# Bazs/structure_from_motion

Hardware: NVIDIA B200
Metric: hyp x point evals/sec (fp64) (higher is better)
Workload: dtype f64

## Files before the change

include/sfm_b200.h:

```cpp
#ifndef SFM_B200_H
#define SFM_B200_H

#include <stdint.h>

#ifdef __cplusplus
extern "C" {
#endif

typedef struct sfm_ctx sfm_ctx;

enum sfm_status {
    SFM_OK = 0,
    SFM_ERR_ARG = -1,
    SFM_ERR_CUDA = -2,
    SFM_ERR_STATE = -3,
    SFM_ERR_NO_DEVICE = -4
};

enum sfm_aggregation { SFM_AGG_SUM = 0, SFM_AGG_SQUARE = 1, SFM_AGG_MEAN = 2, SFM_AGG_RMS = 3 };
enum sfm_selection { SFM_SELECT_MIN_ERROR = 0, SFM_SELECT_MAX_INLIERS = 1, SFM_SELECT_MSAC = 2 };
enum sfm_score_variant { SFM_SCORE_SCREEN = 0, SFM_SCORE_FULL = 1, SFM_SCORE_SCREEN32 = 2, SFM_SCORE_AUTO = 3 };

int sfm_version(void);
const char *sfm_last_error(void);
int sfm_device_count(void);
int sfm_create(int device, sfm_ctx **out);
int sfm_destroy(sfm_ctx *ctx);
int sfm_set_stream(sfm_ctx *ctx, void *cuda_stream);
int sfm_use_default_stream(sfm_ctx *ctx);
int sfm_synchronize(sfm_ctx *ctx);
int sfm_set_score_variant(sfm_ctx *ctx, int variant, int hyps_per_thread, int group);
int sfm_host_alloc(uint64_t bytes, void **out);
int sfm_host_free(void *p);

int sfm_mt_shuffle_table(uint32_t *state625, int64_t n, int64_t h, int32_t *table, int64_t perm_at,
                         int32_t *perm_out);
// ... 22 lines not shown

typedef struct sfm_best {
    double err;
    int64_t index;
    int32_t count_extra;
    int32_t reserved;
    int64_t num_invalid;
    int64_t first_invalid;
    double E[9];
    int32_t sample[8];
} sfm_best;
int sfm_get_best(sfm_ctx *ctx, sfm_best *out);
int sfm_set_winner(sfm_ctx *ctx, int64_t local_index, const double *E);
int sfm_near_ties(sfm_ctx *ctx, double rel_tol, int64_t cap, int64_t *idx_out, int64_t *count);
int sfm_get_rescored(sfm_ctx *ctx, int64_t *count);
int sfm_inlier_mask(sfm_ctx *ctx, double threshold, uint8_t *mask, double *sed);

int sfm_ransac_essential(sfm_ctx *ctx, double threshold, double min_extra, int aggregation,
                         int selection, sfm_best *best, uint8_t *mask, double *sed);

int sfm_fit_homography(sfm_ctx *ctx, double *H_out, uint8_t *valid_out);
int sfm_ransac_homography(sfm_ctx *ctx, double threshold, double min_extra, int aggregation, int selection,
                          sfm_best *best, uint8_t *mask, double *err, int32_t *count_extra_h, double *err_h);
int sfm_homography_mask(sfm_ctx *ctx, const double *H, double threshold, uint8_t *mask, double *err);

typedef struct sfm_poses {
    double R[4][9];
    double t[4][3];
    double sv[3];
    int64_t counts[4];
// ... 107 lines not shown
```

structure_from_motion_b200/_native.py:

```python
from __future__ import annotations

import ctypes as C
import os
import threading

import numpy as np

_HERE = os.path.dirname(os.path.abspath(__file__))
LIB_PATH = os.environ.get("SFM_B200_LIB") or os.path.join(_HERE, "libsfm_b200.so")

AGG = {"sum": 0, "square": 1, "mean": 2, "rms": 3}
SELECT = {"min_error": 0, "max_inliers": 1, "msac": 2}
VARIANT = {"screen": 0, "full": 1, "screen32": 2, "auto": 3}


class NativeUnavailableError(RuntimeError):
    """libsfm_b200.so is missing / not loadable, or there is no B200 to run it on."""


class NativeError(RuntimeError):
    """A C-ABI call returned a non-zero status."""


class Best(C.Structure):
    _fields_ = [("err", C.c_double), ("index", C.c_int64), ("count_extra", C.c_int32),
                ("reserved", C.c_int32), ("num_invalid", C.c_int64), ("first_invalid", C.c_int64),
                ("E", C.c_double * 9), ("sample", C.c_int32 * 8)]

# ... 34 lines not shown
    "sfm_set_table": (C.c_int, [_P, _P, C.c_int64]),
    "sfm_sample_device": (C.c_int, [_P, C.c_uint64, C.c_uint64, C.c_int64, C.c_int64]),
    "sfm_get_table": (C.c_int, [_P, _P, C.c_int64, C.c_int64]),
    "sfm_upload_pairs": (C.c_int, [_P, _P, _P, _P, _P, C.c_int64, C.c_int64, _P]),
    "sfm_upload_pairs_async": (C.c_int, [_P, _P, _P, _P, _P, C.c_int64, C.c_int64, _P]),
    "sfm_upload_pairs_d": (C.c_int, [_P, _P, _P, _P, _P, C.c_int64, C.c_int64, _P]),
    "sfm_get_normalised": (C.c_int, [_P, _P, C.c_int64]),
    "sfm_fit": (C.c_int, [_P, _P, _P, _P]),
    "sfm_set_models": (C.c_int, [_P, _P, _P, C.c_int64]),
    "sfm_get_models": (C.c_int, [_P, C.c_int64, C.c_int64, _P, _P]),
    "sfm_score": (C.c_int, [_P, C.c_double, C.c_double, C.c_int, C.c_int, C.c_int, C.c_int64, _P, _P, _P, _P]),
    "sfm_get_best": (C.c_int, [_P, C.POINTER(Best)]),
    "sfm_set_winner": (C.c_int, [_P, C.c_int64, _P]),
    "sfm_near_ties": (C.c_int, [_P, C.c_double, C.c_int64, _P, C.POINTER(C.c_int64)]),
    "sfm_get_rescored": (C.c_int, [_P, C.POINTER(C.c_int64)]),
    "sfm_inlier_mask": (C.c_int, [_P, C.c_double, _P, _P]),
    "sfm_ransac_essential": (C.c_int, [_P, C.c_double, C.c_double, C.c_int, C.c_int, C.POINTER(Best), _P, _P]),
    "sfm_fit_homography": (C.c_int, [_P, _P, _P]),
    "sfm_ransac_homography": (C.c_int, [_P, C.c_double, C.c_double, C.c_int, C.c_int, C.POINTER(Best), _P, _P, _P, _P]),
    "sfm_homography_mask": (C.c_int, [_P, _P, C.c_double, _P, _P]),
    "sfm_decompose_essential": (C.c_int, [_P, _P, C.POINTER(Poses)]),
    "sfm_recover_pose": (C.c_int, [_P, _P, _P, _P, _P, _P, C.c_int64, C.c_int64, C.c_double, C.POINTER(Poses), _P]),
    "sfm_recover_pose_pixels": (C.c_int, [_P, _P, _P, _P, _P, _P, _P, C.c_int64, C.c_int64, C.c_double,
                                          C.POINTER(Poses), _P]),
    "sfm_triangulate": (C.c_int, [_P, _P, _P, _P, _P, _P, _P, C.c_int64, C.c_int64, _P]),
    "sfm_pose_and_triangulate": (C.c_int, [_P, C.c_double, C.c_double, C.POINTER(Poses), C.c_int64,
                                           C.POINTER(C.c_int64), _P, _P, _P]),
    "sfm_two_view": (C.c_int, [_P, C.c_double, C.c_double, C.c_int, C.c_int, C.c_double, C.POINTER(Best), C.POINTER(Poses),
                               C.c_int64, C.POINTER(C.c_int64), _P, _P, _P, _P, _P]),
    "sfm_two_view_async": (C.c_int, [_P, C.c_double, C.c_double, C.c_int, C.c_int, C.c_double, _P, _P]),
# ... 229 lines not shown
    def set_winner(self, local_index, E=None):
        Ea = None if E is None else _f64(E).reshape(9)
        self._ck(self.lib.sfm_set_winner(self.h, int(local_index), _ptr(Ea)), "sfm_set_winner")

    def near_ties(self, rel_tol=1e-12, cap=64):
        idx = np.empty(cap, dtype=np.int64)
        n = C.c_int64(0)
        self._ck(self.lib.sfm_near_ties(self.h, float(rel_tol), int(cap), _ptr(idx), C.byref(n)), "sfm_near_ties")
        return np.sort(idx[:min(int(n.value), cap)]), int(n.value)

    def rescored(self) -> int:
        n = C.c_int64(0)
        self._ck(self.lib.sfm_get_rescored(self.h, C.byref(n)), "sfm_get_rescored")
        return int(n.value)

    def inlier_mask(self, threshold, want_sed=True):
        mask = np.empty(self.n, dtype=np.uint8)
        sed = np.empty(self.n, dtype=np.float64) if want_sed else None
        self._ck(self.lib.sfm_inlier_mask(self.h, float(threshold), _ptr(mask), _ptr(sed)), "sfm_inlier_mask")
        return mask.astype(bool), sed

    def ransac_essential(self, threshold, min_extra=0.0, aggregation="rms", selection="min_error",
                         want_mask=True, want_sed=True, mask_out=None, sed_out=None):
        b = Best()
        mask = mask_out if mask_out is not None else (np.empty(self.n, dtype=np.uint8) if want_mask else None)
        sed = sed_out if sed_out is not None else (np.empty(self.n, dtype=np.float64) if want_sed else None)
        self._ck(self.lib.sfm_ransac_essential(self.h, float(threshold), float(min_extra), AGG[aggregation],
                                               SELECT[selection], C.byref(b), _ptr(mask), _ptr(sed)),
                 "sfm_ransac_essential")
        return b, mask, sed
# ... 447 lines not shown
```

structure_from_motion_b200/csrc/sfm_api.cu:

```cuda
#include "../../include/sfm_b200.h"

#include <dlfcn.h>

#include <cmath>
#include <cstdarg>
#include <cstdio>
#include <cstdlib>
#include <cstring>
#include <string>
#include <vector>

#include "sfm_device.cuh"
#include "sfm_fit.cuh"
#include "sfm_linalg.cuh"
#include "sfm_score.cuh"
#include "sfm_homography.cuh"
#include "sfm_pose.cuh"
#include "sfm_tail.cuh"
#include "sfm_misc.cuh"
#include "sfm_match.cuh"
#include "sfm_harris.cuh"
#include "sfm_select.cuh"

using namespace sfm;

static_assert(sizeof(Corr) == 32, "Corr must be 32 bytes");
static_assert(sizeof(PoseSet) == sizeof(sfm_poses), "PoseSet/sfm_poses layout mismatch");
static_assert(sizeof(SelectRecord) == SFM_RECORD_BYTES, "SelectRecord / SFM_RECORD_BYTES mismatch");
static_assert(sizeof(ModelScores) == sizeof(sfm_model_scores), "ModelScores / sfm_model_scores layout mismatch");

// ... 54 lines not shown
enum { T_UPLOAD = 0, T_SAMPLE, T_FIT, T_SCORE, T_SELECT, T_MASK, T_POSE, T_TRI, T_COUNT };

}

struct sfm_ctx {
    int device = 0;
    int sm_count = 148;
    cudaStream_t own_stream = nullptr, stream = nullptr;
    Buf raw, pts, offsets, Ks, table, E, valid, eig;
    Buf acc, count_extra, S1, S2, err, blocks, best, invalid, winnerE, spts, bounds, fitflag, record, merged, rows, blockinv;
    Buf m_img, m_feat, m_W, m_ss, m_ok, m_S, m_out;
    Buf h_img, h_gx, h_gy, h_corner, h_alive, h_key, h_idx, h_small, h_xy;
    Buf mask, sed, poses, pass, X, idx, scan, tmp, tailstate, num, winrec, bout;
    Buf planes, hK;
    Buf selstate, selpp;
    long long n = 0, h = 0, npairs = 1;
    long long first_len = 0;
    long long raw_stride = 1;
    bool batched = false, has_pts = false, has_table = false, has_models = false, has_score = false;
    bool models_h = false;
    int hscore_occ = 0;
    bool table_pending = false;
    unsigned long long smp_seed = 0, smp_stream = 0;
    long long smp_offset = 0;
    bool acc_clean = false;
    size_t acc_planes_for = 0;
    double Kstage[9] = {0};
    double hstage[18] = {0};
    double sstage[27] = {0};
    const void* occ_fn[4] = {nullptr, nullptr, nullptr, nullptr};
// ... 157 lines not shown
        c->ev_used[i] = false;
    }
    CU(cudaFuncSetAttribute(k_fit, cudaFuncAttributeMaxDynamicSharedMemorySize,
                            (int)(kFitThreads * kFitSmemDoubles * sizeof(double))));
    *out = c;
    return 0;
}

int sfm_destroy(sfm_ctx* c) {
    if (!c) return 0;
    cudaSetDevice(c->device);
    cudaStreamSynchronize(c->stream);
    Buf* bufs[] = {&c->raw, &c->pts, &c->offsets, &c->Ks, &c->table, &c->E, &c->valid, &c->eig, &c->acc,
                   &c->count_extra, &c->S1, &c->S2, &c->err, &c->blocks, &c->best,
                   &c->invalid, &c->winnerE, &c->record, &c->merged, &c->rows, &c->blockinv, &c->mask, &c->sed, &c->poses, &c->pass, &c->X, &c->idx,
                   &c->planes, &c->hK, &c->selstate, &c->selpp,
                   &c->scan, &c->tmp, &c->gathered, &c->tailstate, &c->num, &c->winrec, &c->bout, &c->spts, &c->bounds, &c->fitflag,
                   &c->m_img, &c->m_feat, &c->m_W, &c->m_ss, &c->m_ok, &c->m_S, &c->m_out,
                   &c->h_img, &c->h_gx, &c->h_gy, &c->h_corner, &c->h_alive, &c->h_key, &c->h_idx, &c->h_small, &c->h_xy};
    for (Buf* b : bufs) b->release();
    for (int i = 0; i < T_COUNT; ++i) {
        cudaEventDestroy(c->ev0[i]);
        cudaEventDestroy(c->ev1[i]);
    }
    sfm_nccl_destroy(c);
    if (c->hpin) cudaFreeHost(c->hpin);
    cudaStreamDestroy(c->own_stream);
    delete c;
    return 0;
}

// ... 5 lines not shown

int sfm_use_default_stream(sfm_ctx* c) {
    if (int r = use(c)) return r;
    c->stream = cudaStreamLegacy;
    return 0;
}

int sfm_synchronize(sfm_ctx* c) {
    if (int r = use(c)) return r;
    CU(cudaStreamSynchronize(c->stream));
    return 0;
}

int sfm_set_score_variant(sfm_ctx* c, int variant, int hpt, int group) {
    if (!c) return fail(SFM_ERR_ARG, "null context");
    if (variant != SFM_SCORE_SCREEN && variant != SFM_SCORE_FULL && variant != SFM_SCORE_SCREEN32 && variant != SFM_SCORE_AUTO)
        return fail(SFM_ERR_ARG, "bad variant %d", variant);
    int nh = hpt ? hpt : c->hpt, ng = group ? group : c->group;
    if (!hpt && (variant == SFM_SCORE_SCREEN32) != (c->variant == SFM_SCORE_SCREEN32)) {
        nh = variant == SFM_SCORE_SCREEN32 ? 4 : 2;
        ng = variant == SFM_SCORE_SCREEN32 ? 8 : 16;
    }
    if (!score_kernel(variant == SFM_SCORE_AUTO ? SFM_SCORE_SCREEN : variant, nh, ng) ||
        (variant == SFM_SCORE_AUTO && !score_kernel(SFM_SCORE_FULL, nh, ng)))
        return fail(SFM_ERR_ARG, "unsupported combination: hyps_per_thread %d, group %d", nh, ng);
    c->variant = variant;
    c->hpt = nh;
    c->group = ng;
    return 0;
}

int sfm_host_alloc(uint64_t bytes, void** out) {
    if (!out) return fail(SFM_ERR_ARG, "out is null");
    CU(cudaMallocHost(out, bytes ? bytes : 1));
    return 0;
}
int sfm_host_free(void* p) {
    if (p) CU(cudaFreeHost(p));
// ... 53 lines not shown

int sfm_get_table(sfm_ctx* c, int32_t* table, int64_t first, int64_t h) {
    if (int r = use(c)) return r;
    if (!c->has_table || first < 0 || h < 0 || first + h > c->h * c->npairs)
        return fail(SFM_ERR_STATE, "no table rows [%lld, %lld)", (long long)first, (long long)(first + h));
    if (int r = ensure_table(c)) return r;
    CU(cudaMemcpyAsync(table, c->table.as<int32_t>() + 8 * first, (size_t)h * 32, cudaMemcpyDeviceToHost, c->stream));
    CU(cudaStreamSynchronize(c->stream));
    return 0;
}

static int normalise_from(sfm_ctx* c, const double* xa, const double* ya, const double* xb, const double* yb,
                          int64_t stride, int64_t n, int64_t max_len) {
    if (int r = c->pts.reserve((size_t)n * sizeof(Corr))) return r;
    if (int r = c->bounds.reserve(16)) return r;
    CU(cudaMemsetAsync(c->bounds.p, 0, 16, c->stream));
    dim3 grid((unsigned)((max_len + 255) / 256), (unsigned)c->npairs);
    k_normalise<<<grid, 256, 0, c->stream>>>(xa, ya, xb, yb, stride, n,
                                             c->batched ? c->offsets.as<long long>() : nullptr,
                                             c->Ks.as<double>(), c->pts.as<Corr>(), c->bounds.as<unsigned long long>());
    return check_launch(c, "k_normalise");
}

static int stage_coords(sfm_ctx* c, double* d, const double* xa, const double* ya, const double* xb, const double* yb,
                        int64_t stride, int64_t n, const double* s[4]) {
    if (stride == 1) {
        const double* src[4] = {xa, ya, xb, yb};
        for (int k = 0; k < 4; ++k)
            CU(cudaMemcpyAsync(d + (size_t)k * n, src[k], (size_t)n * sizeof(double), cudaMemcpyHostToDevice, c->stream));
        s[0] = d; s[1] = d + n; s[2] = d + 2 * n; s[3] = d + 3 * n;
    } else if (stride == 2 && ya == xa + 1 && yb == xb + 1) {
        CU(cudaMemcpyAsync(d, xa, (size_t)n * 2 * sizeof(double), cudaMemcpyHostToDevice, c->stream));
        CU(cudaMemcpyAsync(d + 2 * n, xb, (size_t)n * 2 * sizeof(double), cudaMemcpyHostToDevice, c->stream));
        s[0] = d; s[1] = d + 1; s[2] = d + 2 * n; s[3] = d + 2 * n + 1;
    } else {
        return fail(SFM_ERR_ARG, "unsupported layout: stride must be 1 (four arrays) or 2 (two interleaved [n][2] arrays)");
// ... 31 lines not shown
        const double* src[4] = {xa, ya, xb, yb};
        for (int k = 0; k < 4; ++k) {
            CU(cudaMemcpy2DAsync(d + (size_t)k * n, sizeof(double), src[k], (size_t)stride * sizeof(double),
                                 sizeof(double), (size_t)n, cudaMemcpyDeviceToDevice, c->stream));
            s[k] = d + (size_t)k * n;
        }
        c->raw_stride = stride = 1;
    } else if (int r = stage_raw(c, xa, ya, xb, yb, stride, n, s)) {
        return r;
    }
    if (int r = c->Ks.reserve(9 * sizeof(double))) return r;
    memcpy(c->Khost, K, sizeof c->Khost);
    CU(cudaMemcpyAsync(c->Ks.p, c->Khost, 9 * sizeof(double), cudaMemcpyHostToDevice, c->stream));
    c->n = n;
    if (int r = normalise_from(c, s[0], s[1], s[2], s[3], stride, n, n)) return r;
    c->toc(T_UPLOAD);
    if (sync) CU(cudaStreamSynchronize(c->stream));
    c->has_pts = true;
    c->has_table = c->has_models = c->has_score = false;
    c->table_pending = false;
    c->winner_set = false;
    return 0;
}

int sfm_upload_pairs(sfm_ctx* c, const double* xa, const double* ya, const double* xb, const double* yb,
                     int64_t stride, int64_t n, const double* K) {
    return upload_pairs_impl(c, xa, ya, xb, yb, stride, n, K, false, true);
}

int sfm_upload_pairs_async(sfm_ctx* c, const double* xa, const double* ya, const double* xb, const double* yb,
// ... 199 lines not shown
        if (int r = ensure_table(c)) return r;
    if (agg < 0 || agg > 3) return fail(SFM_ERR_ARG, "bad aggregation %d", agg);
    if (mode < 0 || mode > 2) return fail(SFM_ERR_ARG, "bad selection %d", mode);
    const bool skip_k2 = !(thr >= 0.0) || thr > 1e100;
    const int force_rescore = (thr > 1e100) ? 1 : 0;
    const long long h = c->h, P = c->npairs;
    const int hpt = (c->variant == SFM_SCORE_SCREEN32 && thr > 1e6) ? 2 : c->hpt;
    const int G = (c->variant == SFM_SCORE_SCREEN32 && thr > 1e6) ? 16 : c->group;
    const long long hblocks = (h + 32ll * hpt - 1) / (32ll * hpt);
    const size_t H = (size_t)h * P;
    if (int r = reserve_selection(c, h, P)) return r;
    int e2 = 0;
    if (thr > 0.0 && !skip_k2) (void)frexp(thr, &e2);
    if (e2 < -400) e2 = -400;
    const bool autov = c->variant == SFM_SCORE_AUTO;
    int variant = autov ? SFM_SCORE_SCREEN : c->variant;
    if (variant == SFM_SCORE_SCREEN32 && thr > 1e6) variant = SFM_SCORE_SCREEN;
    const bool f32 = variant == SFM_SCORE_SCREEN32;
    const bool screen = variant != SFM_SCORE_FULL;
    double thr_pre = f32 ? thr * kThr32Factor : (screen ? thr * (1.0 + 1e-9) : thr * (1.0 + 1e-9) + 1e-22);
    if (f32 && thr_pre < 1e-24) thr_pre = 1e-24;
    if (screen && thr_pre < 1e-280) thr_pre = 1e-280;
    const double s_scale = sqrt(thr_pre);
    const double scale1 = ldexp(1.0, 63 - e2), scale2 = ldexp(1.0, 63 - 2 * e2);
    unsigned long long* acc_dev = nullptr;
    {
        const void* fn = score_kernel(variant, hpt, G);
        if (!fn) return fail(SFM_ERR_ARG, "unsupported scoring configuration (variant %d, hpt %d, group %d)", variant, hpt, G);
        const size_t smem_one = (size_t)kScoreWarps * score_warp_smem(hpt, false);
        const size_t smem_two = (size_t)kScoreWarps * score_warp_smem(hpt, true);
        const size_t smem_both = smem_one > smem_two ? smem_one : smem_two;
// ... 15 lines not shown
        if (int r = occupancy(fn, smem, &occ)) return r;
#ifndef SFM_AUTO_SINGLE
#define SFM_AUTO_SINGLE 1
#endif
        const void* fn_auto = nullptr;
        if (autov && SFM_AUTO_SINGLE) {
            if (hpt == 2 && G == 16) fn_auto = reinterpret_cast<const void*>(&k_score_auto<2, 16>);
            if (hpt == 4 && G == 8) fn_auto = reinterpret_cast<const void*>(&k_score_auto<4, 8>);
        }
        if (fn_auto)
            if (int r = occupancy(fn_auto, smem_both, &occ)) return r;
        const void* fn_full = (autov && !fn_auto) ? score_kernel(SFM_SCORE_FULL, hpt, G) : nullptr;
        int occ_full = 0;
        if (fn_full)
            if (int r = occupancy(fn_full, smem_two, &occ_full)) return r;
        const long long grid_blocks = (long long)c->sm_count * occ;
        constexpr int items_per_warp = 32;
        const ItemSplit sp = split_items(grid_blocks * kScoreWarps * items_per_warp, hblocks * P, max_len, kTile);
        const long long chunk = sp.chunk, nsplit = sp.nsplit;
        const long long total_items = hblocks * nsplit * P;
        if (int r = c->acc.reserve(H * kAccWords * 8 + acc_tail_bytes(P))) return r;
        const long long npts = c->n;
        if (f32) { if (int r = c->spts.reserve((size_t)npts * sizeof(Corr32))) return r; }
        else if (screen) { if (int r = c->spts.reserve((size_t)npts * sizeof(Corr))) return r; }
        ScoreArgs a;
        a.pts = c->pts.as<Corr>();
        a.spts = screen ? c->spts.p : c->pts.p;
        a.bounds = c->bounds.as<double>();
        a.s = s_scale;
        a.kappa_coef = kKappaCoef * (1.0 + thr);
// ... 6 lines not shown
        a.thr = thr;
        a.thr_pre = thr_pre;
        a.scale1 = scale1;
        a.scale2 = scale2;
        a.sums = sums;
        a.chunk = chunk;
        a.hblocks = (int)hblocks;
        a.nsplit = (int)nsplit;
        a.total_items = total_items;
        a.htotal = (long long)H;
        a.acc = c->acc.as<unsigned long long>();
        a.work_counter = reinterpret_cast<unsigned*>(a.acc + H * kAccWords);
        char* tailp = reinterpret_cast<char*>(a.acc + H * kAccWords);
        a.mode_flag = autov ? reinterpret_cast<const int*>(tailp + 32) : nullptr;
        acc_dev = a.acc;
        c->tic(T_SCORE);
        if (int r = clear_acc(c, H, P)) return r;
        if (f32 && !skip_k2) {
            k_screen_pts32<<<(unsigned)((npts + 255) / 256), 256, 0, c->stream>>>(c->pts.as<Corr>(), npts, 1.0 / s_scale,
                                                                                  reinterpret_cast<Corr32*>(c->spts.p));
            if (int r = check_launch(c, "k_screen_pts32")) return r;
        }
        else if (screen && !skip_k2) {
            PilotArgs pa;
            pa.E = c->E.as<double>();
            pa.h = h;
            pa.plen = c->batched ? c->first_len : c->n;
            pa.thr_pre = thr_pre;
            pa.counters = reinterpret_cast<unsigned*>(tailp + 16);
            pa.mode_flag = autov ? reinterpret_cast<int*>(tailp + 32) : nullptr;
            CU(chain_launch(c, k_screen_pts64, dim3((unsigned)((npts + 255) / 256)), dim3(256), 0, c->pts.as<Corr>(), npts,
                            1.0 / s_scale, reinterpret_cast<Corr*>(c->spts.p), pa));
            if (int r = check_launch(c, "k_screen_pts64")) return r;
        }
        const long long want_blocks = (total_items + kScoreWarps - 1) / kScoreWarps;
        const long long launch_blocks = grid_blocks < want_blocks ? grid_blocks : want_blocks;
        void* kargs[] = {(void*)&a};
        if (!skip_k2 && fn_auto) {
            ScoreArgs a2 = a;
            a2.thr_pre = thr * (1.0 + 1e-9) + 1e-22;
            a2.spts = c->pts.p;
            void* kargs2[] = {(void*)&a, (void*)&a2};
            CU(chain_launch_ptr(c, fn_auto, dim3((unsigned)launch_blocks), dim3(kScoreThreads), smem_both, kargs2));
            if (int r = check_launch(c, "k_score_auto")) return r;
        } else if (!skip_k2) {
            CU(chain_launch_ptr(c, fn, dim3((unsigned)launch_blocks), dim3(kScoreThreads), smem, kargs));
            if (int r = check_launch(c, "k_score")) return r;
            if (fn_full) {
                ScoreArgs a2 = a;
                a2.thr_pre = thr * (1.0 + 1e-9) + 1e-22;
                a2.spts = c->pts.p;
                const long long gb2 = (long long)c->sm_count * occ_full;
                const long long lb2 = gb2 < want_blocks ? gb2 : want_blocks;
                void* kargs2[] = {(void*)&a2};
                CU(chain_launch_ptr(c, fn_full, dim3((unsigned)lb2), dim3(kScoreThreads), smem_two, kargs2));
                if (int r = check_launch(c, "k_score")) return r;
            }
        }
        c->toc(T_SCORE);
    }

    return finalise_launch(c, MODEL_E, thr, min_extra, agg, mode, use_table, idx_offset, sums, e2, force_rescore, acc_dev);
}

int sfm_score(sfm_ctx* c, double thr, double min_extra, int agg, int mode, int use_table, int64_t idx_offset,
              int32_t* count_extra, double* S1, double* S2, double* err) {
    if (int r = use(c)) return r;
    if (c->batched) return fail(SFM_ERR_STATE, "sfm_score is a single-pair call; use sfm_batch_ransac");
    if (int r = score_launch(c, thr, min_extra, agg, mode, use_table != 0, idx_offset, c->n, S1 || S2)) return r;
    const size_t H = (size_t)c->h;
    if (count_extra) CU(cudaMemcpyAsync(count_extra, c->count_extra.p, H * 4, cudaMemcpyDeviceToHost, c->stream));
    if (S1) CU(cudaMemcpyAsync(S1, c->S1.p, H * 8, cudaMemcpyDeviceToHost, c->stream));
    if (S2) CU(cudaMemcpyAsync(S2, c->S2.p, H * 8, cudaMemcpyDeviceToHost, c->stream));
    if (err) CU(cudaMemcpyAsync(err, c->err.p, H * 8, cudaMemcpyDeviceToHost, c->stream));
    CU(cudaStreamSynchronize(c->stream));
    return 0;
// ... 38 lines not shown
    if (int r = c->tmp.reserve((size_t)cap * 8 + 16)) return r;
    unsigned* cnt = c->tmp.as<unsigned>();
    long long* out = reinterpret_cast<long long*>(c->tmp.as<char>() + 16);
    CU(cudaMemsetAsync(cnt, 0, 16, c->stream));
    const int blocks = (int)((c->h + 255) / 256 < 4 * c->sm_count ? (c->h + 255) / 256 : 4 * c->sm_count);
    k_near_ties<<<blocks, 256, 0, c->stream>>>(c->err.as<double>(), c->h, c->record.as<SelectRecord>(), rel_tol, (int)cap, out, cnt);
    if (int r = check_launch(c, "k_near_ties")) return r;
    if (int r = ensure_pinned(c, (size_t)cap * 8 + 16)) return r;
    CU(cudaMemcpyAsync(c->hpin, c->tmp.p, (size_t)cap * 8 + 16, cudaMemcpyDeviceToHost, c->stream));
    CU(cudaStreamSynchronize(c->stream));
    unsigned n;
    memcpy(&n, c->hpin, 4);
    *count = n;
    const int64_t take = n < (unsigned)cap ? n : cap;
    memcpy(idx_out, (char*)c->hpin + 16, (size_t)take * 8);
    return 0;
}

int sfm_get_rescored(sfm_ctx* c, int64_t* count) {
    if (int r = use(c)) return r;
    if (!count) return fail(SFM_ERR_ARG, "null argument");
    if (!c->rescored_dev) return fail(SFM_ERR_STATE, "no scoring call yet");
    if (int r = ensure_pinned(c, 8)) return r;
    CU(cudaMemcpyAsync(c->hpin, c->rescored_dev, 8, cudaMemcpyDeviceToHost, c->stream));
    CU(cudaStreamSynchronize(c->stream));
    unsigned long long v;
    memcpy(&v, c->hpin, 8);
    *count = (int64_t)v;
    return 0;
}
// ... 1147 lines not shown
```

Before: 1029 billion.

## Add spatial-cell bounding-box pruning path for essential-matrix scoring

Adds a cells scoring variant. Points are sorted into spatial cells of 64 with a k-d-style radix-sort partition, and each cell gets a bounding box. A new kernel skips whole (hypothesis, cell) pairs whose box provably lies outside the threshold and evaluates only the surviving pairs, using a warp ring buffer and shared accumulators. In AUTO mode the path is enabled for large point sets after the first score, gated on a low pilot inlier rate. This adds one-time sort and bbox cost per upload, plus extra kernel launches and complexity.

Result: faster. 1093 billion, median of 6 (+6.3%).

```diff
diff --git a/include/sfm_b200.h b/include/sfm_b200.h
--- a/include/sfm_b200.h
+++ b/include/sfm_b200.h
@@ -19,7 +19,9 @@
 
 enum sfm_aggregation { SFM_AGG_SUM = 0, SFM_AGG_SQUARE = 1, SFM_AGG_MEAN = 2, SFM_AGG_RMS = 3 };
 enum sfm_selection { SFM_SELECT_MIN_ERROR = 0, SFM_SELECT_MAX_INLIERS = 1, SFM_SELECT_MSAC = 2 };
-enum sfm_score_variant { SFM_SCORE_SCREEN = 0, SFM_SCORE_FULL = 1, SFM_SCORE_SCREEN32 = 2, SFM_SCORE_AUTO = 3 };
+enum sfm_score_variant {
+    SFM_SCORE_SCREEN = 0, SFM_SCORE_FULL = 1, SFM_SCORE_SCREEN32 = 2, SFM_SCORE_AUTO = 3, SFM_SCORE_CELLS = 4
+};
 
 int sfm_version(void);
 const char *sfm_last_error(void);
@@ -72,6 +74,7 @@
 int sfm_set_winner(sfm_ctx *ctx, int64_t local_index, const double *E);
 int sfm_near_ties(sfm_ctx *ctx, double rel_tol, int64_t cap, int64_t *idx_out, int64_t *count);
 int sfm_get_rescored(sfm_ctx *ctx, int64_t *count);
+int sfm_get_cell_evals(sfm_ctx *ctx, int64_t *evaluated, int64_t *pairs);
 int sfm_inlier_mask(sfm_ctx *ctx, double threshold, uint8_t *mask, double *sed);
 
 int sfm_ransac_essential(sfm_ctx *ctx, double threshold, double min_extra, int aggregation,
diff --git a/structure_from_motion_b200/_native.py b/structure_from_motion_b200/_native.py
--- a/structure_from_motion_b200/_native.py
+++ b/structure_from_motion_b200/_native.py
@@ -11,7 +11,7 @@
 
 AGG = {"sum": 0, "square": 1, "mean": 2, "rms": 3}
 SELECT = {"min_error": 0, "max_inliers": 1, "msac": 2}
-VARIANT = {"screen": 0, "full": 1, "screen32": 2, "auto": 3}
+VARIANT = {"screen": 0, "full": 1, "screen32": 2, "auto": 3, "cells": 4}
 
 
 class NativeUnavailableError(RuntimeError):
@@ -76,6 +76,7 @@
     "sfm_set_winner": (C.c_int, [_P, C.c_int64, _P]),
     "sfm_near_ties": (C.c_int, [_P, C.c_double, C.c_int64, _P, C.POINTER(C.c_int64)]),
     "sfm_get_rescored": (C.c_int, [_P, C.POINTER(C.c_int64)]),
+    "sfm_get_cell_evals": (C.c_int, [_P, C.POINTER(C.c_int64), C.POINTER(C.c_int64)]),
     "sfm_inlier_mask": (C.c_int, [_P, C.c_double, _P, _P]),
     "sfm_ransac_essential": (C.c_int, [_P, C.c_double, C.c_double, C.c_int, C.c_int, C.POINTER(Best), _P, _P]),
     "sfm_fit_homography": (C.c_int, [_P, _P, _P]),
@@ -335,6 +336,11 @@
         self._ck(self.lib.sfm_get_rescored(self.h, C.byref(n)), "sfm_get_rescored")
         return int(n.value)
 
+    def cell_evaluations(self):
+        ev, pairs = C.c_int64(0), C.c_int64(0)
+        self._ck(self.lib.sfm_get_cell_evals(self.h, C.byref(ev), C.byref(pairs)), "sfm_get_cell_evals")
+        return int(ev.value), int(pairs.value)
+
     def inlier_mask(self, threshold, want_sed=True):
         mask = np.empty(self.n, dtype=np.uint8)
         sed = np.empty(self.n, dtype=np.float64) if want_sed else None
diff --git a/structure_from_motion_b200/csrc/sfm_api.cu b/structure_from_motion_b200/csrc/sfm_api.cu
--- a/structure_from_motion_b200/csrc/sfm_api.cu
+++ b/structure_from_motion_b200/csrc/sfm_api.cu
@@ -10,10 +10,13 @@
 #include <string>
 #include <vector>
 
+#include <cub/device/device_radix_sort.cuh>
+
 #include "sfm_device.cuh"
 #include "sfm_fit.cuh"
 #include "sfm_linalg.cuh"
 #include "sfm_score.cuh"
+#include "sfm_cells.cuh"
 #include "sfm_homography.cuh"
 #include "sfm_pose.cuh"
 #include "sfm_tail.cuh"
@@ -98,6 +101,12 @@
     Buf mask, sed, poses, pass, X, idx, scan, tmp, tailstate, num, winrec, bout;
     Buf planes, hK;
     Buf selstate, selpp;
+    Buf ckey, cperm, cbb, cbox, cpts, ctemp;
+    bool cells_ready = false;
+    int scores_since_upload = 0;
+    long long ncells = 0;
+    long long cell_pairs = 0;
+    const unsigned long long* cell_evals_dev = nullptr;
     long long n = 0, h = 0, npairs = 1;
     long long first_len = 0;
     long long raw_stride = 1;
@@ -285,7 +294,7 @@
     Buf* bufs[] = {&c->raw, &c->pts, &c->offsets, &c->Ks, &c->table, &c->E, &c->valid, &c->eig, &c->acc,
                    &c->count_extra, &c->S1, &c->S2, &c->err, &c->blocks, &c->best,
                    &c->invalid, &c->winnerE, &c->record, &c->merged, &c->rows, &c->blockinv, &c->mask, &c->sed, &c->poses, &c->pass, &c->X, &c->idx,
-                   &c->planes, &c->hK, &c->selstate, &c->selpp,
+                   &c->planes, &c->hK, &c->selstate, &c->selpp, &c->ckey, &c->cperm, &c->cbb, &c->cbox, &c->cpts, &c->ctemp,
                    &c->scan, &c->tmp, &c->gathered, &c->tailstate, &c->num, &c->winrec, &c->bout, &c->spts, &c->bounds, &c->fitflag,
                    &c->m_img, &c->m_feat, &c->m_W, &c->m_ss, &c->m_ok, &c->m_S, &c->m_out,
                    &c->h_img, &c->h_gx, &c->h_gy, &c->h_corner, &c->h_alive, &c->h_key, &c->h_idx, &c->h_small, &c->h_xy};
@@ -321,14 +330,15 @@
 
 int sfm_set_score_variant(sfm_ctx* c, int variant, int hpt, int group) {
     if (!c) return fail(SFM_ERR_ARG, "null context");
-    if (variant != SFM_SCORE_SCREEN && variant != SFM_SCORE_FULL && variant != SFM_SCORE_SCREEN32 && variant != SFM_SCORE_AUTO)
+    if (variant != SFM_SCORE_SCREEN && variant != SFM_SCORE_FULL && variant != SFM_SCORE_SCREEN32 && variant != SFM_SCORE_AUTO &&
+        variant != SFM_SCORE_CELLS)
         return fail(SFM_ERR_ARG, "bad variant %d", variant);
     int nh = hpt ? hpt : c->hpt, ng = group ? group : c->group;
     if (!hpt && (variant == SFM_SCORE_SCREEN32) != (c->variant == SFM_SCORE_SCREEN32)) {
         nh = variant == SFM_SCORE_SCREEN32 ? 4 : 2;
         ng = variant == SFM_SCORE_SCREEN32 ? 8 : 16;
     }
-    if (!score_kernel(variant == SFM_SCORE_AUTO ? SFM_SCORE_SCREEN : variant, nh, ng) ||
+    if (!score_kernel((variant == SFM_SCORE_AUTO || variant == SFM_SCORE_CELLS) ? SFM_SCORE_SCREEN : variant, nh, ng) ||
         (variant == SFM_SCORE_AUTO && !score_kernel(SFM_SCORE_FULL, nh, ng)))
         return fail(SFM_ERR_ARG, "unsupported combination: hyps_per_thread %d, group %d", nh, ng);
     c->variant = variant;
@@ -412,12 +422,59 @@
                           int64_t stride, int64_t n, int64_t max_len) {
     if (int r = c->pts.reserve((size_t)n * sizeof(Corr))) return r;
     if (int r = c->bounds.reserve(16)) return r;
+    c->cells_ready = false;
+    c->scores_since_upload = 0;
     CU(cudaMemsetAsync(c->bounds.p, 0, 16, c->stream));
     dim3 grid((unsigned)((max_len + 255) / 256), (unsigned)c->npairs);
     k_normalise<<<grid, 256, 0, c->stream>>>(xa, ya, xb, yb, stride, n,
                                              c->batched ? c->offsets.as<long long>() : nullptr,
                                              c->Ks.as<double>(), c->pts.as<Corr>(), c->bounds.as<unsigned long long>());
     return check_launch(c, "k_normalise");
+}
+
+static bool cells_wanted(const sfm_ctx* c) {
+    return !c->batched && (c->variant == SFM_SCORE_CELLS ||
+                           (c->variant == SFM_SCORE_AUTO && c->n >= kCellsMinPoints && c->scores_since_upload > 0));
+}
+static int ensure_cells(sfm_ctx* c) {
+    if (c->cells_ready) return 0;
+    const long long n = c->n, nc = (n + kCell - 1) / kCell;
+    int levels = 0;
+    while ((1ll << levels) < nc) ++levels;
+    size_t temp = 0;
+    CU(cub::DeviceRadixSort::SortPairs(nullptr, temp, (const unsigned long long*)nullptr, (unsigned long long*)nullptr,
+                                       (const int*)nullptr, (int*)nullptr, (int)n, 0, kCellKeyBits + levels, c->stream));
+    if (int r = c->ckey.reserve((size_t)n * 16)) return r;
+    if (int r = c->cperm.reserve((size_t)n * 8)) return r;
+    if (int r = c->cbb.reserve((size_t)nc * 64)) return r;
+    if (int r = c->cbox.reserve((size_t)nc * sizeof(CellBox))) return r;
+    if (int r = c->cpts.reserve((size_t)nc * kCell * sizeof(Corr))) return r;
+    if (int r = c->ctemp.reserve(temp)) return r;
+    unsigned long long* const kin = c->ckey.as<unsigned long long>();
+    unsigned long long* const kout = kin + n;
+    int* const vin = c->cperm.as<int>();
+    int* const vout = vin + n;
+    const int* perm = nullptr;
+    const unsigned gp = (unsigned)((nc * kCell + 255) / 256), gn = (unsigned)((n + 255) / 256);
+    unsigned long long* bb = c->cbb.as<unsigned long long>();
+    for (int l = 0; l < levels; ++l) {
+        CU(cudaMemsetAsync(bb, 0, ((size_t)1 << l) * 64, c->stream));
+        k_cell_bbox<<<gp, 256, 0, c->stream>>>(c->pts.as<Corr>(), perm, n, nc, l, bb);
+        if (int r = check_launch(c, "k_cell_bbox")) return r;
+        k_cell_keys<<<gn, 256, 0, c->stream>>>(c->pts.as<Corr>(), perm, n, nc, l, bb, kin, vin);
+        if (int r = check_launch(c, "k_cell_keys")) return r;
+        size_t t = temp;
+        CU(cub::DeviceRadixSort::SortPairs(c->ctemp.p, t, kin, kout, vin, vout, (int)n, 0, kCellKeyBits + l, c->stream));
+        perm = vout;
+    }
+    CU(cudaMemsetAsync(bb, 0, (size_t)nc * 64, c->stream));
+    k_cell_bbox<<<gp, 256, 0, c->stream>>>(c->pts.as<Corr>(), perm, n, nc, -1, bb);
+    if (int r = check_launch(c, "k_cell_bbox")) return r;
+    k_cell_finish<<<gp, 256, 0, c->stream>>>(c->pts.as<Corr>(), perm, n, nc, bb, c->cbox.as<CellBox>(), c->cpts.as<Corr>());
+    if (int r = check_launch(c, "k_cell_finish")) return r;
+    c->ncells = nc;
+    c->cells_ready = true;
+    return 0;
 }
 
 static int stage_coords(sfm_ctx* c, double* d, const double* xa, const double* ya, const double* xb, const double* yb,
@@ -479,6 +536,8 @@
     CU(cudaMemcpyAsync(c->Ks.p, c->Khost, 9 * sizeof(double), cudaMemcpyHostToDevice, c->stream));
     c->n = n;
     if (int r = normalise_from(c, s[0], s[1], s[2], s[3], stride, n, n)) return r;
+    if (cells_wanted(c))
+        if (int r = ensure_cells(c)) return r;
     c->toc(T_UPLOAD);
     if (sync) CU(cudaStreamSynchronize(c->stream));
     c->has_pts = true;
@@ -708,7 +767,9 @@
     if (thr > 0.0 && !skip_k2) (void)frexp(thr, &e2);
     if (e2 < -400) e2 = -400;
     const bool autov = c->variant == SFM_SCORE_AUTO;
-    int variant = autov ? SFM_SCORE_SCREEN : c->variant;
+    const bool cells = !skip_k2 && cells_wanted(c);
+    const bool cells_only = cells && c->variant == SFM_SCORE_CELLS;
+    int variant = (autov || c->variant == SFM_SCORE_CELLS) ? SFM_SCORE_SCREEN : c->variant;
     if (variant == SFM_SCORE_SCREEN32 && thr > 1e6) variant = SFM_SCORE_SCREEN;
     const bool f32 = variant == SFM_SCORE_SCREEN32;
     const bool screen = variant != SFM_SCORE_FULL;
@@ -754,6 +815,10 @@
         int occ_full = 0;
         if (fn_full)
             if (int r = occupancy(fn_full, smem_two, &occ_full)) return r;
+        const size_t smem_cells = (size_t)kScoreWarps * sizeof(CellWarpSmem);
+        int occ_cells = 0;
+        if (cells)
+            if (int r = occupancy(reinterpret_cast<const void*>(&k_score_cells), smem_cells, &occ_cells)) return r;
         const long long grid_blocks = (long long)c->sm_count * occ;
         constexpr int items_per_warp = 32;
         const ItemSplit sp = split_items(grid_blocks * kScoreWarps * items_per_warp, hblocks * P, max_len, kTile);
@@ -790,6 +855,10 @@
         char* tailp = reinterpret_cast<char*>(a.acc + H * kAccWords);
         a.mode_flag = autov ? reinterpret_cast<const int*>(tailp + 32) : nullptr;
         acc_dev = a.acc;
+        if (cells)
+            if (int r = ensure_cells(c)) return r;
+        c->cell_pairs = cells ? h * c->ncells : 0;
+        c->cell_evals_dev = reinterpret_cast<const unsigned long long*>(tailp + 40);
         c->tic(T_SCORE);
         if (int r = clear_acc(c, H, P)) return r;
         if (f32 && !skip_k2) {
@@ -797,7 +866,7 @@
                                                                                   reinterpret_cast<Corr32*>(c->spts.p));
             if (int r = check_launch(c, "k_screen_pts32")) return r;
         }
-        else if (screen && !skip_k2) {
+        else if (screen && !skip_k2 && !cells_only) {
             PilotArgs pa;
             pa.E = c->E.as<double>();
             pa.h = h;
@@ -812,14 +881,31 @@
         const long long want_blocks = (total_items + kScoreWarps - 1) / kScoreWarps;
         const long long launch_blocks = grid_blocks < want_blocks ? grid_blocks : want_blocks;
         void* kargs[] = {(void*)&a};
-        if (!skip_k2 && fn_auto) {
+        if (cells) {
+            CellArgs ca;
+            ca.a = a;
+            ca.a.hblocks = (int)((h + 63) / 64);
+            ca.a.total_items = (long long)ca.a.hblocks * ((c->ncells + kCellsPerItem - 1) / kCellsPerItem);
+            ca.cpts = c->cpts.as<Corr>();
+            ca.box = c->cbox.as<CellBox>();
+            ca.ncells = c->ncells;
+            ca.inv_s = 1.0 / s_scale;
+            ca.pilot = autov ? reinterpret_cast<const unsigned long long*>(tailp + 16) : nullptr;
+            ca.mode_flag = autov ? reinterpret_cast<int*>(tailp + 32) : nullptr;
+            ca.evaluated = reinterpret_cast<unsigned long long*>(tailp + 40);
+            const long long gb = (long long)c->sm_count * occ_cells;
+            const long long wb = (ca.a.total_items + kScoreWarps - 1) / kScoreWarps;
+            CU(chain_launch(c, k_score_cells, dim3((unsigned)(gb < wb ? gb : wb)), dim3(kScoreThreads), smem_cells, ca));
+            if (int r = check_launch(c, "k_score_cells")) return r;
+        }
+        if (!skip_k2 && !cells_only && fn_auto) {
             ScoreArgs a2 = a;
             a2.thr_pre = thr * (1.0 + 1e-9) + 1e-22;
             a2.spts = c->pts.p;
             void* kargs2[] = {(void*)&a, (void*)&a2};
             CU(chain_launch_ptr(c, fn_auto, dim3((unsigned)launch_blocks), dim3(kScoreThreads), smem_both, kargs2));
             if (int r = check_launch(c, "k_score_auto")) return r;
-        } else if (!skip_k2) {
+        } else if (!skip_k2 && !cells_only) {
             CU(chain_launch_ptr(c, fn, dim3((unsigned)launch_blocks), dim3(kScoreThreads), smem, kargs));
             if (int r = check_launch(c, "k_score")) return r;
             if (fn_full) {
@@ -836,6 +922,7 @@
         c->toc(T_SCORE);
     }
 
+    c->scores_since_upload += 1;
     return finalise_launch(c, MODEL_E, thr, min_extra, agg, mode, use_table, idx_offset, sums, e2, force_rescore, acc_dev);
 }
 
@@ -904,6 +991,21 @@
     *count = n;
     const int64_t take = n < (unsigned)cap ? n : cap;
     memcpy(idx_out, (char*)c->hpin + 16, (size_t)take * 8);
+    return 0;
+}
+
+int sfm_get_cell_evals(sfm_ctx* c, int64_t* evaluated, int64_t* pairs) {
+    if (int r = use(c)) return r;
+    if (!evaluated || !pairs) return fail(SFM_ERR_ARG, "null argument");
+    *evaluated = *pairs = 0;
+    if (!c->cell_evals_dev || !c->cell_pairs) return 0;
+    if (int r = ensure_pinned(c, 8)) return r;
+    CU(cudaMemcpyAsync(c->hpin, c->cell_evals_dev, 8, cudaMemcpyDeviceToHost, c->stream));
+    CU(cudaStreamSynchronize(c->stream));
+    unsigned long long v;
+    memcpy(&v, c->hpin, 8);
+    *evaluated = (int64_t)v;
+    *pairs = c->cell_pairs;
     return 0;
 }
 
diff --git a/structure_from_motion_b200/csrc/sfm_cells.cuh b/structure_from_motion_b200/csrc/sfm_cells.cuh
--- /dev/null
+++ b/structure_from_motion_b200/csrc/sfm_cells.cuh
@@ -0,0 +1,354 @@
+#pragma once
+#include <cfloat>
+
+#include "sfm_score.cuh"
+
+namespace sfm {
+
+constexpr int kCell = 64;
+constexpr int kCellsPerItem = 16;
+constexpr int kCellKeyBits = 16;
+constexpr long long kCellsMinPoints = 32768;
+constexpr double kPilotCellsBelow = 0.03;
+enum { MODE_CELLS = 3 };
+static_assert(kCell * kCellsPerItem <= kMaxItemPoints, "an item must stay inside the 32-bit chunk sums");
+
+struct __align__(16) CellBox {
+    double c[4], w[4];
+};
+
+__device__ __forceinline__ unsigned long long dkey(double x) {
+    const unsigned long long u = (unsigned long long)__double_as_longlong(x);
+    return (u >> 63) ? ~u : (u | 0x8000000000000000ull);
+}
+__device__ __forceinline__ double dunkey(unsigned long long k) {
+    return __longlong_as_double((long long)((k >> 63) ? (k & 0x7fffffffffffffffull) : ~k));
+}
+__host__ __device__ __forceinline__ long long cell_node(long long cell, int level, long long nc) {
+    return (((cell + 1) << level) - 1) / nc;
+}
+
+__global__ void __launch_bounds__(256) k_cell_bbox(const Corr* __restrict__ pts, const int* __restrict__ perm, long long n,
+                                                   long long nc, int level, unsigned long long* __restrict__ bb) {
+    const long long i = blockIdx.x * (long long)blockDim.x + threadIdx.x;
+    const long long cell = i / kCell;
+    if (cell >= nc) return;
+    const bool live = i < n;
+    Corr p = {0.0, 0.0, 0.0, 0.0};
+    if (live) p = pts[perm ? perm[i] : i];
+    const double v[4] = {p.xa, p.ya, p.xb, p.yb};
+    unsigned long long k[8];
+#pragma unroll
+    for (int d = 0; d < 4; ++d) {
+        k[d] = live ? ~dkey(v[d]) : 0ull;
+        k[4 + d] = live ? dkey(v[d]) : 0ull;
+    }
+#pragma unroll
+    for (int s = 16; s > 0; s >>= 1)
+#pragma unroll
+        for (int d = 0; d < 8; ++d) {
+            const unsigned long long o = __shfl_xor_sync(0xffffffffu, k[d], s);
+            k[d] = o > k[d] ? o : k[d];
+        }
+    if ((threadIdx.x & 31) == 0) {
+        const long long node = level < 0 ? cell : cell_node(cell, level, nc);
+#pragma unroll
+        for (int d = 0; d < 8; ++d) atomicMax(bb + 8 * node + d, k[d]);
+    }
+}
+
+__global__ void __launch_bounds__(256) k_cell_keys(const Corr* __restrict__ pts, const int* __restrict__ perm, long long n,
+                                                   long long nc, int level, const unsigned long long* __restrict__ bb,
+                                                   unsigned long long* __restrict__ key, int* __restrict__ val) {
+    const long long i = blockIdx.x * (long long)blockDim.x + threadIdx.x;
+    if (i >= n) return;
+    const long long node = cell_node(i / kCell, level, nc);
+    const unsigned long long* b = bb + 8 * node;
+    int axis = 0;
+    double lo = dunkey(~b[0]), width = dunkey(b[4]) - lo, best = width;
+#pragma unroll
+    for (int d = 1; d < 4; ++d) {
+        const double l = dunkey(~b[d]), w = dunkey(b[4 + d]) - l;
+        if (w > best) { best = w; axis = d; lo = l; }
+    }
+    const int src = perm ? perm[i] : (int)i;
+    const Corr p = pts[src];
+    const double x = axis == 0 ? p.xa : (axis == 1 ? p.ya : (axis == 2 ? p.xb : p.yb));
+    const double t = (x - lo) / best;
+    const double top = (double)((1u << kCellKeyBits) - 1);
+    const unsigned q = t >= 1.0 ? (unsigned)top : (t > 0.0 ? (unsigned)(t * (top + 1.0)) : 0u);
+    key[i] = ((unsigned long long)node << kCellKeyBits) | (q > (unsigned)top ? (unsigned)top : q);
+    val[i] = src;
+}
+
+__global__ void __launch_bounds__(256) k_cell_finish(const Corr* __restrict__ pts, const int* __restrict__ perm, long long n,
+                                                     long long nc, const unsigned long long* __restrict__ bb,
+                                                     CellBox* __restrict__ box, Corr* __restrict__ cpts) {
+    const long long i = blockIdx.x * (long long)blockDim.x + threadIdx.x;
+    if (i >= nc * kCell) return;
+    Corr p = {0.0, 0.0, 0.0, 0.0};
+    if (i < n) p = pts[perm ? perm[i] : i];
+    cpts[i] = p;
+    if (i % kCell) return;
+    const long long cell = i / kCell;
+    CellBox cb;
+#pragma unroll
+    for (int d = 0; d < 4; ++d) {
+        const double lo = dunkey(~bb[8 * cell + d]), hi = dunkey(bb[8 * cell + 4 + d]);
+        const double c = __dadd_rn(__dmul_rn(lo, 0.5), __dmul_rn(hi, 0.5));
+        const double a = __dsub_ru(hi, c), b = __dsub_ru(c, lo);
+        double w = a >= b ? a : b;
+        if (!(w <= DBL_MAX) || !(c == c)) w = __longlong_as_double(0x7ff0000000000000LL);
+        cb.c[d] = c;
+        cb.w[d] = w;
+    }
+    box[cell] = cb;
+}
+
+struct CellArgs {
+    ScoreArgs a;
+    const Corr* cpts;
+    const CellBox* box;
+    long long ncells;
+    double inv_s;
+    const unsigned long long* pilot;
+    int* mode_flag;
+    unsigned long long* evaluated;
+};
+
+struct alignas(128) CellWarpSmem {
+    double model[64][10];
+    unsigned sacc[2][kAccWords][32];
+    unsigned ring[kRing];
+    unsigned char list[64];
+};
+
+__device__ __forceinline__ double cell_screen(const double* m, double xa, double ya, double xb, double yb) {
+    const double2* r = reinterpret_cast<const double2*>(m);
+    const double2 m0 = r[0], m1 = r[1], m2 = r[2], m3 = r[3], m4 = r[4];
+    double t0 = fma(yb, m1.y, m3.x);
+    double t1 = fma(yb, m2.x, m3.y);
+    double t2 = fma(yb, m2.y, m4.x);
+    t0 = fma(xb, m0.x, t0);
+    t1 = fma(xb, m0.y, t1);
+    t2 = fma(xb, m1.x, t2);
+    t2 = fma(ya, t1, t2);
+    t2 = fma(xa, t0, t2);
+    t1 = fma(t1, t1, m4.y);
+    t1 = fma(t0, t0, t1);
+    return fma(t2, t2, -t1);
+}
+
+__device__ __forceinline__ double abs_hi(double lo, double hi) { return hi >= -lo ? hi : -lo; }
+
+struct ScaledBox {
+    double ac0, ac1, wa0, wa1, bc0, bc1, wb0, wb1, w00, w01, w10, w11;
+};
+__device__ __forceinline__ bool cell_pruned(const double (&e)[9], double kap, const ScaledBox& x) {
+    double L[3], U[3];
+#pragma unroll
+    for (int j = 0; j < 3; ++j) {
+        L[j] = __fma_rd(x.bc0, e[j], __fma_rd(x.bc1, e[3 + j], e[6 + j]));
+        U[j] = __fma_ru(x.bc0, e[j], __fma_ru(x.bc1, e[3 + j], e[6 + j]));
+    }
+    const double P0 = __fma_rd(x.ac0, e[0], __fma_rd(x.ac1, e[1], e[2])), Q0 = __fma_ru(x.ac0, e[0], __fma_ru(x.ac1, e[1], e[2]));
+    const double P1 = __fma_rd(x.ac0, e[3], __fma_rd(x.ac1, e[4], e[5])), Q1 = __fma_ru(x.ac0, e[3], __fma_ru(x.ac1, e[4], e[5]));
+    const bool p0 = x.ac0 >= 0.0, p1 = x.ac1 >= 0.0;
+    const double rlo = __fma_rd(x.ac0, p0 ? L[0] : U[0], __fma_rd(x.ac1, p1 ? L[1] : U[1], L[2]));
+    const double rhi = __fma_ru(x.ac0, p0 ? U[0] : L[0], __fma_ru(x.ac1, p1 ? U[1] : L[1], U[2]));
+    const double ar = rlo > 0.0 ? rlo : (rhi < 0.0 ? -rhi : 0.0);
+    const double g0 = abs_hi(L[0], U[0]), g1 = abs_hi(L[1], U[1]);
+    const double cross = __fma_ru(fabs(e[0]), x.w00, __fma_ru(fabs(e[1]), x.w01, __fma_ru(fabs(e[3]), x.w10, __dmul_ru(fabs(e[4]), x.w11))));
+    const double dev = __fma_ru(g0, x.wa0, __fma_ru(g1, x.wa1, __fma_ru(abs_hi(P0, Q0), x.wb0, __fma_ru(abs_hi(P1, Q1), x.wb1, cross))));
+    const double lr = __dsub_rd(ar, dev);
+    const double m0 = __fma_ru(fabs(e[0]), x.wb0, __fma_ru(fabs(e[3]), x.wb1, g0));
+    const double m1 = __fma_ru(fabs(e[1]), x.wb0, __fma_ru(fabs(e[4]), x.wb1, g1));
+    const double mhi = __fma_ru(m0, m0, __fma_ru(m1, m1, kap));
+    return lr > 0.0 && __dmul_rd(lr, lr) > mhi;
+}
+
+__device__ __forceinline__ ScaledBox scale_box(const CellBox& b, double inv_s, bool& ok) {
+    ScaledBox x;
+    double ca[2], wa[2];
+#pragma unroll
+    for (int d = 0; d < 2; ++d) {
+        const double lo = __dmul_rd(__dsub_rd(b.c[d], b.w[d]), inv_s), hi = __dmul_ru(__dadd_ru(b.c[d], b.w[d]), inv_s);
+        ca[d] = __dadd_rn(__dmul_rn(lo, 0.5), __dmul_rn(hi, 0.5));
+        const double u = __dsub_ru(hi, ca[d]), v = __dsub_ru(ca[d], lo);
+        wa[d] = u >= v ? u : v;
+    }
+    x.ac0 = ca[0]; x.ac1 = ca[1]; x.wa0 = wa[0]; x.wa1 = wa[1];
+    x.bc0 = b.c[2]; x.bc1 = b.c[3]; x.wb0 = b.w[2]; x.wb1 = b.w[3];
+    x.w00 = __dmul_ru(x.wb0, x.wa0); x.w01 = __dmul_ru(x.wb0, x.wa1);
+    x.w10 = __dmul_ru(x.wb1, x.wa0); x.w11 = __dmul_ru(x.wb1, x.wa1);
+    ok = fabs(x.ac0) <= DBL_MAX && fabs(x.ac1) <= DBL_MAX && x.wa0 <= DBL_MAX && x.wa1 <= DBL_MAX &&
+         fabs(x.bc0) <= DBL_MAX && fabs(x.bc1) <= DBL_MAX && x.wb0 <= DBL_MAX && x.wb1 <= DBL_MAX;
+    return x;
+}
+
+__global__ void __launch_bounds__(kScoreThreads, 4) k_score_cells(const CellArgs ca) {
+    chain_enter();
+    const ScoreArgs& a = ca.a;
+    if (ca.pilot) {
+        const unsigned long long t = *ca.pilot;
+        const double rate = (unsigned)t ? (double)(t >> 32) / (double)(unsigned)t : 0.0;
+        if (!(rate < kPilotCellsBelow)) return;
+        if (blockIdx.x == 0 && threadIdx.x == 0) *ca.mode_flag = MODE_CELLS;
+    }
+    extern __shared__ __align__(128) unsigned char cell_smem[];
+    const unsigned full = 0xffffffffu;
+    const int lane = threadIdx.x & 31;
+    const int warp = __shfl_sync(full, (int)(threadIdx.x >> 5), 0);
+    const unsigned lt = lanemask_lt();
+    CellWarpSmem& ws = reinterpret_cast<CellWarpSmem*>(cell_smem)[warp];
+#pragma unroll
+    for (int j = 0; j < 2; ++j)
+#pragma unroll
+        for (int k = 0; k < kAccWords; ++k) ws.sacc[j][k][lane] = 0;
+    __syncwarp();
+    unsigned head = 0, tail = 0;
+    const double ab2 = a.bounds[0] * a.bounds[1] * a.kappa_coef;
+    const long long hblocks = a.hblocks;
+
+    for (;;) {
+        unsigned item = 0;
+        if (lane == 0) item = atomicAdd(a.work_counter, 1u);
+        item = __shfl_sync(full, item, 0);
+        if (item >= a.total_items) break;
+        const long long hyp_w = (long long)(item % (unsigned)hblocks) * 64;
+        const long long cell0 = (long long)(item / (unsigned)hblocks) * kCellsPerItem;
+        const int ncell = (int)(ca.ncells - cell0 < kCellsPerItem ? ca.ncells - cell0 : kCellsPerItem);
+        const long long begin = cell0 * kCell;
+        const ModelRow* Rw = a.rows + hyp_w;
+
+        double e[2][9], kap[2];
+        bool real[2], prunable[2];
+#pragma unroll
+        for (int j = 0; j < 2; ++j) {
+            const long long hyp = hyp_w + 32 * j + lane;
+            real[j] = hyp < a.h;
+            double v[9], f2 = 0.0;
+#pragma unroll
+            for (int k = 0; k < 9; ++k) {
+                v[k] = real[j] ? a.E[9 * hyp + k] : 0.0;
+                f2 = fma(v[k], v[k], f2);
+            }
+#pragma unroll
+            for (int k = 0; k < 9; ++k) e[j][k] = (k % 3) != 2 ? v[k] * a.s : v[k];
+            kap[j] = real[j] ? f2 * ab2 : -1.0;
+            prunable[j] = f2 <= DBL_MAX;
+            double2* mp = reinterpret_cast<double2*>(&ws.model[32 * j + lane][0]);
+            mp[0] = make_double2(e[j][0], e[j][1]);
+            mp[1] = make_double2(e[j][2], e[j][3]);
+            mp[2] = make_double2(e[j][4], e[j][5]);
+            mp[3] = make_double2(e[j][6], e[j][7]);
+            mp[4] = make_double2(e[j][8], kap[j]);
+        }
+        __syncwarp();
+
+        auto drain = [&]() {
+            const unsigned navail = tail - head;
+            const bool act = (unsigned)lane < navail;
+            const unsigned en = act ? ws.ring[(head + lane) & (kRing - 1)] : 0u;
+            const unsigned hl = en >> 16, pos = en & 0xffffu;
+            const int slot = (int)(hl >> 5), owner = (int)(hl & 31u);
+            const ModelRow* er = Rw + hl;
+            const double4 r0 = er->a, r1 = er->b;
+            const double eo[9] = {r0.x, r0.y, r0.z, r0.w, r1.x, r1.y, r1.z, r1.w, er->c.x};
+            const Corr c = ca.cpts[begin + pos];
+            const double sv = sed_exact(eo, c.xa, c.ya, c.xb, c.yb);
+            if (act && (sv <= a.thr)) {
+                unsigned ch[kChunks];
+                unsigned* dst = &ws.sacc[slot][0][owner];
+                atomicAdd(dst, 1u);
+                if (a.sums & SUM_S1) {
+                    chunks21(sv, a.scale1, ch);
+#pragma unroll
+                    for (int kk = 0; kk < kChunks; ++kk) atomicAdd(dst + 32 * (1 + kk), ch[kk]);
+                }
+                if (a.sums & SUM_S2) {
+                    chunks21(__dmul_rn(sv, sv), a.scale2, ch);
+#pragma unroll
+                    for (int kk = 0; kk < kChunks; ++kk) atomicAdd(dst + 32 * (1 + kChunks + kk), ch[kk]);
+                }
+            }
+            head += navail < 32u ? navail : 32u;
+            __syncwarp();
+        };
+
+        unsigned long long evals = 0;
+        Corr nxa = ca.cpts[begin + lane], nxb = ca.cpts[begin + 32 + lane];
+        for (int k = 0; k < ncell; ++k) {
+            const Corr pa = nxa, pb = nxb;
+            if (k + 1 < ncell) {
+                nxa = ca.cpts[begin + (long long)(k + 1) * kCell + lane];
+                nxb = ca.cpts[begin + (long long)(k + 1) * kCell + 32 + lane];
+            }
+            bool boxok;
+            const ScaledBox x = scale_box(ca.box[cell0 + k], ca.inv_s, boxok);
+            bool keep[2];
+#pragma unroll
+            for (int j = 0; j < 2; ++j) keep[j] = real[j] && !(boxok && prunable[j] && cell_pruned(e[j], kap[j], x));
+            const unsigned k0 = __ballot_sync(full, keep[0]), k1 = __ballot_sync(full, keep[1]);
+            if (keep[0]) ws.list[__popc(k0 & lt)] = (unsigned char)lane;
+            if (keep[1]) ws.list[__popc(k0) + __popc(k1 & lt)] = (unsigned char)(32 + lane);
+            const int nl = __popc(k0) + __popc(k1);
+            evals += (unsigned long long)nl;
+            __syncwarp();
+            const long long base = begin + (long long)k * kCell;
+            const bool la = base + lane < a.n, lb = base + 32 + lane < a.n;
+            const double xaa = pa.xa * ca.inv_s, yaa = pa.ya * ca.inv_s;
+            const double xab = pb.xa * ca.inv_s, yab = pb.ya * ca.inv_s;
+            unsigned long long ha = 0ull, hb = 0ull;
+            for (int i = 0; i < nl; ++i) {
+                const unsigned h = ws.list[i];
+                const double* m = &ws.model[h][0];
+                const double da = cell_screen(m, xaa, yaa, pa.xb, pa.yb);
+                const double db = cell_screen(m, xab, yab, pb.xb, pb.yb);
+                ha |= (unsigned long long)((unsigned)sign_word(da) >> 31) << h;
+                hb |= (unsigned long long)((unsigned)sign_word(db) >> 31) << h;
+            }
+            if (!la) ha = 0ull;
+            if (!lb) hb = 0ull;
+            __syncwarp();
+            const unsigned rel0 = (unsigned)(k * kCell + lane);
+            unsigned vote;
+            while ((vote = __ballot_sync(full, (ha | hb) != 0ull)) != 0u) {
+                unsigned en = 0u;
+                if (ha) {
+                    en = ((unsigned)(__ffsll((long long)ha) - 1) << 16) | rel0;
+                    ha &= ha - 1ull;
+                } else if (hb) {
+                    en = ((unsigned)(__ffsll((long long)hb) - 1) << 16) | (rel0 + 32u);
+                    hb &= hb - 1ull;
+                }
+                if ((vote >> lane) & 1u) ws.ring[(tail + __popc(vote & lt)) & (kRing - 1)] = en;
+                tail += __popc(vote);
+                __syncwarp();
+                if (tail - head >= 32u) drain();
+            }
+        }
+        while (tail != head) drain();
+        if (lane == 0) atomicAdd(ca.evaluated, evals);
+#pragma unroll
+        for (int j = 0; j < 2; ++j) {
+            const unsigned cnt = ws.sacc[j][0][lane];
+            if (cnt) {
+                unsigned long long* dst = a.acc + hyp_w + 32 * j + lane;
+                atomicAdd(dst, (unsigned long long)cnt);
+                ws.sacc[j][0][lane] = 0;
+#pragma unroll
+                for (int k = 1; k < kAccWords; ++k) {
+                    const unsigned v = ws.sacc[j][k][lane];
+                    if (v) {
+                        atomicAdd(dst + (long long)k * a.htotal, (unsigned long long)v);
+                        ws.sacc[j][k][lane] = 0;
+                    }
+                }
+            }
+        }
+        __syncwarp();
+    }
+}
+
+}
```
